# chenkovsky/aha

Hardware: AMD Instinct MI355X
Metric: input GB/s scanned + M-hits/s, 100k-pattern AC over 1 GiB UTF-8 corpus (higher is better)
Workload: dtype u8

## Files before the change

### aha_amd/csrc/scan_unit.hip

```cpp
#include <hip/hip_runtime.h>

#include "automaton.hpp"
#include "devcommon.hpp"
#include "image.hpp"
#include "unit.hpp"

namespace aha {

namespace {

constexpr int kUPiece = 16;
constexpr int kUWin = 3 * kUPiece;
constexpr int kURow = kUWin + 4;
constexpr int kUWave = 64 * kURow;

__device__ __forceinline__ uint4 load16(const uint8_t *text, int64_t g, int64_t N) {
  uint4 v = make_uint4(0, 0, 0, 0);
  if (g >= 0 && g + 16 <= N) {
    v = *reinterpret_cast<const uint4 *>(text + g);
  } else if (g >= 0 && g < N) {
    uint32_t w0 = 0, w1 = 0, w2 = 0, w3 = 0;
#pragma unroll 1
    for (int j = 0; j < 16 && g + j < N; j++) {
      const uint32_t b = (uint32_t)text[g + j] << ((j & 3) * 8);
      w0 |= (j >> 2) == 0 ? b : 0u;
      w1 |= (j >> 2) == 1 ? b : 0u;
      w2 |= (j >> 2) == 2 ? b : 0u;
      w3 |= (j >> 2) == 3 ? b : 0u;
    }
    v = make_uint4(w0, w1, w2, w3);
  }
  return v;
}

__device__ __forceinline__ uint64_t wballot(bool p) { return __builtin_amdgcn_ballot_w64(p); }
__device__ __forceinline__ bool wany(bool p) { return __builtin_amdgcn_ballot_w64(p) != 0ull; }
__device__ __forceinline__ bool wall(bool p) { return __builtin_amdgcn_ballot_w64(!p) == 0ull; }

__host__ __device__ inline size_t u_lds_rows(uint32_t n_syms) {
  return (size_t)(kUTabWords + ((n_syms + 3u) & ~3u)) * 4 + (size_t)(kV2Threads / 64) * kUWave + 16;
}
__host__ __device__ inline size_t u_lds(uint32_t n_syms) {
  return u_lds_rows(n_syms) + (size_t)(kV2Threads / 64) * 64 * 12;
}

template <bool CHARS, int BB, bool HB>
__global__ __launch_bounds__(kV2Threads) void ku_traverse(UnitDev U, V2Args M) {
  extern __shared__ __attribute__((aligned(16))) uint8_t smem[];
  if (M.cursor[1] >= 16ull) return;
  uint32_t *tabw = reinterpret_cast<uint32_t *>(smem);
  uint32_t *rlw = tabw + kUTabWords;
  const uint32_t n_root = (U.n_syms + 3u) & ~3u;
  for (uint32_t i = threadIdx.x; i < kUTabWords; i += kV2Threads) tabw[i] = U.tables[i];
  for (uint32_t i = threadIdx.x; i < n_root; i += kV2Threads) rlw[i] = i < U.n_syms ? U.root[i] : 0u;
  __syncthreads();
  const uint32_t *rl = rlw;
  const uint4 *t0a = reinterpret_cast<const uint4 *>(tabw + kUT0a);
  const uint2 *t0b = reinterpret_cast<const uint2 *>(tabw + kUT0b);
  const uint8_t *tabb = reinterpret_cast<const uint8_t *>(tabw);
  uint8_t *in_base = smem + (size_t)(kUTabWords + n_root) * 4;
  const int lane = threadIdx.x & 63, wave = threadIdx.x >> 6;
  uint8_t *inl = in_base + wave * kUWave + lane * kURow;
  const uint32_t *row = reinterpret_cast<const uint32_t *>(inl);
  typedef uint32_t v3u __attribute__((ext_vector_type(3)));
  const uint32_t wbo = (uint32_t)u_lds_rows(U.n_syms) + (uint32_t)wave * (64u * 12u);
  const uint2 *slots = U.slots;
  const int64_t N = (int64_t)M.n_bytes;
  const uint64_t D = M.n_docs;
  const int64_t S = (int64_t)M.S;
  const int rounds = (int)(M.S / kUPiece);
  const int warm = U.max_len > 1 ? (int)U.max_len - 1 : 0;
  const int R = (warm + kUPiece - 1) / kUPiece;

  const uint64_t n_tiles = (M.n_chunks + kV2Threads - 1) / kV2Threads;
  for (uint64_t tile = blockIdx.x; tile < n_tiles; tile += gridDim.x) {
    const uint64_t chunk = tile * kV2Threads + threadIdx.x;
    const uint32_t ev_stride = M.ev_stride;
    const bool live = chunk < M.n_chunks;
    const int64_t a = (int64_t)chunk * S;
    const int64_t e = live ? min(a + S, N) : a;
    uint64_t dn = 0;
    int64_t nb = INT64_MAX, doc_start = a, pos = e;
    uint32_t wfill = 0, wout = 0;
    const uint64_t wchunk0 = tile * kV2Threads + (uint64_t)wave * 64;
    uint32_t *wreg = M.evg + wchunk0 * M.ev_stride * 3;
    const uint32_t wcap = (uint32_t)min<uint64_t>(64, M.n_chunks > wchunk0 ? M.n_chunks - wchunk0 : 0) * M.ev_stride;
    uint32_t hits = 0;
    uint32_t lead_total = 0;
    uint32_t lc = 0, lc_exact = 0;
    uint32_t E = 0, seq = 0;
    uint32_t pc = 0;
    uint4 q1 = make_uint4(0, 0, 0, 0), q2 = q1, q3 = q1;
    uint32_t w[13] = {0, 0, 0, 0, 0, 0, 0, 0, 0, 0, 0, 0, 0};
    if (live) {
      dn = first_boundary(M.doc_off, D, (uint64_t)a);
      nb = (int64_t)M.doc_off[dn];
      pos = a;
      if (nb != a) {
        doc_start = (int64_t)M.doc_off[dn - 1];
        pos = a - min<int64_t>(a - doc_start, warm);
        if (CHARS) M.chunk_doc0[chunk] = (uint32_t)(dn - 1);
      } else if (CHARS) {
        M.chunk_doc0[chunk] = (uint32_t)dn;
      }
    }

    for (int r = -((R + 3) / 4) * 4 - 2; r <= rounds; r++) {
      const int64_t pb = a + (int64_t)r * kUPiece;
      const int64_t pl = pb + 2 * kUPiece;
      const int64_t pend = min(pb + kUWin, e);
      {
        uint4 v;
        if ((pl & 63) == 0) {
          v = load16(M.text, pl, N);
          q1 = load16(M.text, pl + 16, N);
          q2 = load16(M.text, pl + 32, N);
          q3 = load16(M.text, pl + 48, N);
        } else {
          v = q1;
          q1 = q2;
          q2 = q3;
        }
#pragma unroll
        for (int i = 0; i < 9; i++) w[i] = w[i + 4];
        w[9] = v.x;
        w[10] = v.y;
        w[11] = v.z;
        w[12] = v.w;
        uint32_t *dst = reinterpret_cast<uint32_t *>(inl);
#pragma unroll
        for (int i = 0; i < 13; i++) dst[i] = w[i];
      }
      const bool need = live && pos < pend;
      if (!wany(need)) continue;
      uint32_t rel = kURow, lim = 0;
      if (need) {
        rel = (uint32_t)(pos - pb + 4);
        lim = (uint32_t)(pend - pb + 4);
      }
      uint32_t nb_rel = (nb >= pb - 4 && nb <= pb + kUWin) ? (uint32_t)(nb - pb + 4) : ~0u;
      const uint32_t n_rel = (N - pb) <= (int64_t)kUWin ? (uint32_t)max<int64_t>(N - pb + 4, 0) : ~0u;
      const int32_t a_rel = (int32_t)max<int64_t>(a - pb + 4, -128);
      const int32_t e_rel = (int32_t)min<int64_t>(e - pb + 4, 128);
      int32_t docrel = (int32_t)(pb - 4 - doc_start);

      for (;;) {
        const bool bnd = rel < lim && rel == nb_rel;
        if (wany(bnd)) {
          if (bnd) {
            const int64_t here = pb - 4 + rel;
            do {
              M.doc_ev_rank[dn] = seq;
              M.doc_hit_rank[dn] = hits;
              if (CHARS) M.doc_lead_rank[dn] = lead_total;
              dn++;
              nb = dn <= D ? (int64_t)M.doc_off[dn] : INT64_MAX;
            } while (nb == here);
            asm volatile("" : "+v"(nb));
            nb_rel = (nb <= pb + kUWin) ? (uint32_t)(nb - pb + 4) : ~0u;
            E = 0;
            pc = 0;
            lc = 0;
            lc_exact = 1;
            doc_start = here;
            docrel = -(int32_t)rel;
          }
        }
        uint32_t lim2 = min(lim, nb_rel);
        const uint32_t dend = min(nb_rel, n_rel);
        auto decode = [&](uint32_t at, uint32_t &o_code, uint32_t &o_L, bool &o_later) {
          const uint32_t lo = row[at >> 2], hi = row[(at >> 2) + 1];
          const uint32_t w4 = __builtin_amdgcn_alignbyte(hi, lo, at & 3u);
          const uint32_t b0 = w4 & 0xFFu;
          const uint4 q0 = t0a[b0];
          const uint2 q1 = t0b[b0];
          const uint32_t s1 = *reinterpret_cast<const uint32_t *>(tabb + q0.x + ((w4 >> 6) & 0x3FCu));
          const uint32_t s2 = *reinterpret_cast<const uint32_t *>(tabb + q0.y + ((w4 >> 14) & 0x3FCu));
          const uint32_t sum = q0.z + s1 + s2;
          const uint32_t want = q1.y;
          const bool in_doc = at + want <= dend;
          o_later = in_doc & at + want > (uint32_t)kURow;
          const bool whole = in_doc & sum < kUPoison;
          const bool o_good = whole & (sum - q0.w) < q1.x;
          o_L = whole ? want : 1u;
          if (CHARS) o_L |= (b0 & 0xC0u) != 0x80u ? 0x100u : 0u;
          o_code = o_good ? sum - kUBias : 0u;
        };
        uint32_t code, L;
        {
          bool later;
          decode(min(rel, (uint32_t)kURow), code, L, later);
          lim2 = later ? min(lim2, rel) : lim2;
          lim = later ? min(lim, rel) : lim;
        }
        bool all_left = false;
        for (;;) {
          const bool act = rel < lim2;
          all_left = wall(rel >= (uint32_t)(4 + kUPiece) || rel >= lim);
          if (all_left || !wany(act)) break;
          auto trip = [&]() -> uint32_t {
            uint32_t evc = 0;
            const bool good = code != 0u;
            const uint32_t Bq = u_child(E, BB);
            const bool hdr = u_hdr_pending(E);
            const bool grp = Bq >= U.big_lo & code >= U.n_low & !hdr;
            uint32_t se = grp ? (code >> 5) + U.g0 : code;
            se = hdr ? 0u : se;
            const uint32_t fc = BB == 22 ? (code & 7u) : min(code & 7u, 6u);
            const bool probe = act & good & (((E | 0x20000000u) >> ((uint32_t)BB + fc)) & 1u) != 0u & Bq != 0u;
            unsigned long long enw = 0;
            uint32_t hdw = 0;
            {
              const uint2 *ap = slots + (probe ? (Bq ^ se) : 0u);
              asm volatile("global_load_dwordx2 %0, %1, off" : "=v"(enw) : "v"(ap) : "memory");
              if (HB) {
                const uint2 *hp = slots + ((act & u_nfr(E) & !u_f1(E)) ? Bq : 0u);
                asm volatile("global_load_dword %0, %1, off" : "=v"(hdw) : "v"(hp) : "memory");
              }
            }
            if (act) {
              uint32_t n_code, n_L;
              bool n_later;
              const uint32_t Lb = CHARS ? (L & 0xFFu) : L;
              decode(rel + Lb, n_code, n_L, n_later);
              const uint32_t rt = rl[code];
              const uint32_t rf = rl[pc];
              if (HB)
                asm volatile("s_waitcnt vmcnt(0)" : "+v"(enw), "+v"(hdw) : : "memory");
              else
                asm volatile("s_waitcnt vmcnt(0)" : "+v"(enw) : : "memory");
              const uint32_t enx = (uint32_t)enw, eny = (uint32_t)(enw >> 32);
              const bool symhit = probe & u_sym(eny) == se & !grp;
              const bool hit = symhit & !hdr;
              const bool redir = grp & probe & ((enx >> (code & 31u)) & 1u) != 0u;
              const uint32_t rE = (__builtin_popcount(enx & ~(~0u << (code & 31u))) + eny ^ code) | u_all_filter(BB);
              const bool viaroot = !symhit & !redir & (!u_nfr(E) | !good);
              const uint32_t ft = u_f1(E) ? (rf & 0x7FFFFFFFu) : (HB ? hdw : (Bq | u_all_filter(BB) | 0x20000000u));
              uint32_t missE = viaroot ? rt : ft;
              missE = redir ? rE : missE;
              E = symhit ? enx : missE;
              const bool consumed = hit | viaroot;
              const bool end = consumed & u_end(E);
              const uint32_t c4 = hit ? u_c4(eny) : 1u;
              pc = consumed ? code : pc;
              const uint32_t adv = consumed ? Lb : 0u;
              if (CHARS) {
                const uint32_t isl = (consumed & (int32_t)rel >= a_rel) ? (L >> 8) : 0u;
                lc += isl;
                lead_total += isl;
              }
              rel += adv;
              const bool park = consumed & n_later;
              lim2 = park ? rel : lim2;
              lim = park ? rel : lim;
              code = consumed ? n_code : code;
              L = consumed ? n_L : L;
              const int32_t last = (int32_t)rel - 1;
              evc = (end & last >= a_rel & last < e_rel) ? c4 : 0u;
            }
            return evc;
          };
          const uint32_t evc = trip();
          const uint64_t evm = wballot(evc != 0u);
          if (evm) {
            const bool ev = evc != 0u;
            const uint32_t my = wfill + __builtin_amdgcn_mbcnt_hi((uint32_t)(evm >> 32), __builtin_amdgcn_mbcnt_lo((uint32_t)evm, 0u));
            const uint32_t rx = u_rec_x(u_child(E, BB), (uint32_t)lane, evc, BB), rz = u_rec_z(hits, evc, BB);
            const uint32_t ry = CHARS ? ((lc << 1) | lc_exact) : (uint32_t)(docrel + (int32_t)rel);
            if (ev && my < 64u) {
              uint32_t *d = reinterpret_cast<uint32_t *>(smem + (wbo + __umul24(my, 12u)));
              d[0] = rx;
              d[1] = ry;
              d[2] = rz;
            }
            const uint32_t kp = __popcll(evm);
            if (wfill + kp >= 64u) {
              const uint32_t *q = reinterpret_cast<const uint32_t *>(smem + (wbo + __umul24((uint32_t)lane, 12u)));
              const v3u r = {q[0], q[1], q[2]};
#ifndef AHA_KU_LAB_NOFLUSH
              if (wout + 64u <= wcap) *reinterpret_cast<v3u *>(wreg + (size_t)(wout + lane) * 3) = r;
#else
              if (wout + 64u == 0xFFFFFFF0u) *reinterpret_cast<v3u *>(wreg + (size_t)(wout + lane) * 3) = r;
#endif
              wout += 64u;
              if (ev && my >= 64u) {
                uint32_t *d = reinterpret_cast<uint32_t *>(smem + (wbo + __umul24(my - 64u, 12u)));
                d[0] = rx;
                d[1] = ry;
                d[2] = rz;
              }
            }
            wfill = (wfill + kp) & 63u;
            seq += ev ? 1u : 0u;
            hits += evc;
          }
        }
        if (all_left || !wany(rel < lim)) break;
      }
      if (need) pos = pb - 4 + rel;
    }
    {
      const uint32_t *q = reinterpret_cast<const uint32_t *>(smem + (wbo + __umul24((uint32_t)lane, 12u)));
      const v3u r = {q[0], q[1], q[2]};
      if ((uint32_t)lane < wfill && wout + (uint32_t)lane < wcap) *reinterpret_cast<v3u *>(wreg + (size_t)(wout + lane) * 3) = r;
    }
    if (live) {
      M.ev_cnt[chunk] = seq;
      if (seq > ev_stride) M.cursor[1] = 2ull;
      if (CHARS) M.lead_cnt[chunk] = lead_total;
      M.chunk_hits[chunk] = hits;
      if (e == N) {
        while (dn <= D) {
          M.doc_ev_rank[dn] = seq;
          M.doc_hit_rank[dn] = hits;
          if (CHARS) M.doc_lead_rank[dn] = lead_total;
          dn++;
        }
      }
    }
  }
}

constexpr int kRgThreads = 256, kRgPer = 4, kRgBlock = kRgThreads * kRgPer, kRgSubs = kRgBlock / 64;
__global__ __launch_bounds__(kRgThreads) void ku_regroup(DevAut A, V2Args M) {
  __shared__ uint2 s_sorted[kRgBlock];
  __shared__ uint8_t s_lane[kRgBlock];
  __shared__ uint32_t s_cnt[kRgSubs][64], s_part[kRgThreads / 64][64];
  __shared__ uint32_t s_start[64], s_tot[64], s_run[64], s_hits[64];
  if (M.cursor[1]) return;
  const int lane = threadIdx.x & 63, wv = threadIdx.x >> 6;
  const uint64_t n_groups = (M.n_chunks + 63) / 64;
  const uint32_t stride = M.ev_stride;
  const uint32_t bb = M.unit_bb, bmask = (1u << bb) - 1u;
  for (uint64_t g = blockIdx.x; g < n_groups; g += gridDim.x) {
    __syncthreads();
    if (wv == 0) {
      s_run[lane] = 0;
      s_hits[lane] = 0;
    }
    const uint64_t c = g * 64 + lane;
    uint32_t total = c < M.n_chunks ? min(M.ev_cnt[c], stride) : 0u;
#pragma unroll
    for (int d = 32; d >= 1; d >>= 1) total += __shfl_xor(total, d, 64);
    const uint32_t *src = M.evg + g * 64 * stride * 3;
    uint2 *dst = M.evd + g * 64 * stride;
    uint2 nxt[kRgPer];
    uint32_t xn[kRgPer];
#pragma unroll
    for (int q = 0; q < kRgPer; q++) {
      const uint32_t i = q * kRgThreads + threadIdx.x;
      nxt[q] = i < total ? make_uint2(src[(size_t)i * 3], src[(size_t)i * 3 + 1]) : make_uint2(0, 0);
    }
#pragma unroll
    for (int q = 0; q < kRgPer; q++) xn[q] = (uint32_t)(q * kRgThreads) + threadIdx.x < total ? A.end_info[nxt[q].x & bmask] : 0u;
    for (uint32_t i0 = 0; i0 < total; i0 += kRgBlock) {
      uint2 rec[kRgPer];
      uint32_t x[kRgPer], rank[kRgPer], l[kRgPer];
      bool live[kRgPer];
#pragma unroll
      for (int q = 0; q < kRgPer; q++) {
        const uint32_t i = i0 + q * kRgThreads + threadIdx.x;
        live[q] = i < total;
        rec[q] = nxt[q];
        x[q] = xn[q];
        nxt[q] = i + kRgBlock < total ? make_uint2(src[(size_t)(i + kRgBlock) * 3], src[(size_t)(i + kRgBlock) * 3 + 1])
                                      : make_uint2(0, 0);
      }
#pragma unroll
      for (int q = 0; q < kRgPer; q++) {
        l[q] = (rec[q].x >> bb) & 63u;
        uint64_t same = __ballot(live[q]), mine = same;
#pragma unroll
        for (int b = 0; b < 6; b++) {
          const uint64_t bal = __ballot(live[q] & ((l[q] >> b) & 1u) != 0u);
          same &= ((l[q] >> b) & 1u) ? bal : ~bal;
          mine &= ((lane >> b) & 1) ? bal : ~bal;
        }
        rank[q] = __popcll(same & ((1ull << lane) - 1ull));
        s_cnt[q * (kRgThreads / 64) + wv][lane] = __popcll(mine);
      }
      __syncthreads();
      {
        uint32_t acc = 0;
#pragma unroll
        for (int r = 0; r < kRgSubs / (kRgThreads / 64); r++) {
          const uint32_t v = s_cnt[wv * (kRgSubs / (kRgThreads / 64)) + r][lane];
          s_cnt[wv * (kRgSubs / (kRgThreads / 64)) + r][lane] = acc;
          acc += v;
        }
        s_part[wv][lane] = acc;
      }
      __syncthreads();
      if (wv == 0) {
        uint32_t acc = 0;
#pragma unroll
        for (int w2 = 0; w2 < kRgThreads / 64; w2++) {
          const uint32_t v = s_part[w2][lane];
          s_part[w2][lane] = acc;
          acc += v;
        }
        s_tot[lane] = acc;
        s_start[lane] = wave_incl_scan(acc) - acc;
      }
      __syncthreads();
#pragma unroll
      for (int q = 0; q < kRgPer; q++) {
        if (live[q]) {
          const uint32_t sb = q * (kRgThreads / 64) + wv;
          const uint32_t p = s_start[l[q]] + s_part[sb / (kRgSubs / (kRgThreads / 64))][l[q]] + s_cnt[sb][l[q]] + rank[q];
          uint32_t cnt = x[q] >> 24;
          if (cnt == 255u) cnt = A.key_cnt[A.chain ? A.chain[x[q] & 0xFFFFFFu].y : (x[q] & 0xFFFFFFu)];
          s_sorted[p] = make_uint2(x[q], rec[q].y);
          s_lane[p] = (uint8_t)l[q];
          if (cnt) atomicAdd(&s_hits[l[q]], cnt);
        }
      }
      __syncthreads();
#pragma unroll
      for (int q = 0; q < kRgPer; q++)
        xn[q] = i0 + kRgBlock + (uint32_t)(q * kRgThreads) + threadIdx.x < total ? A.end_info[nxt[q].x & bmask] : 0u;
#pragma unroll
      for (int q = 0; q < kRgPer; q++) asm volatile("" : "+v"(xn[q]));
      const uint32_t nb = min(total - i0, (uint32_t)kRgBlock);
#pragma unroll
      for (int q = 0; q < kRgPer; q++) {
        const uint32_t p = q * kRgThreads + threadIdx.x;
        if (p < nb) {
          const uint32_t lp = s_lane[p];
          const uint32_t at = s_run[lp] + (p - s_start[lp]);
          if (at < stride) dst[(uint64_t)lp * stride + at] = s_sorted[p];
        }
      }
      __syncthreads();
      if (wv == 0) s_run[lane] += s_tot[lane];
    }
    __syncthreads();
    if (wv == 0 && c < M.n_chunks) M.chunk_hits[c] = s_hits[lane];
  }
}

constexpr int kXgThreads = 1024, kXgPer = 1, kXgBlock = kXgThreads * kXgPer, kXgStage = 1536;
constexpr int kXgCacheBits = 11;
template <bool CHARS>
__global__ __launch_bounds__(kXgThreads) void ku_expand_groups(const uint2 *uend, DevAut A, V2Args M) {
  __shared__ uint32_t s_hs[kXgStage], s_he[kXgStage], s_hk[kXgStage];
  __shared__ uint8_t s_hl[kXgStage];
  __shared__ uint32_t s_tot[2][64], s_start[64], s_run[64], s_all;
  __shared__ uint64_t s_base[64];
  __shared__ uint32_t s_adj[64];
  __shared__ unsigned long long s_cache[1 << kXgCacheBits];
  if (M.cursor[1]) return;
  const int lane = threadIdx.x & 63, wv = threadIdx.x >> 6;
  const uint64_t n_groups = (M.n_chunks + 63) / 64;
  const uint32_t stride = M.ev_stride;
  const uint32_t bb = M.unit_bb, bmask = (1u << bb) - 1u;
  for (uint32_t i = threadIdx.x; i < (1u << kXgCacheBits); i += kXgThreads) s_cache[i] = 0ull;
  for (uint64_t g = blockIdx.x; g < n_groups; g += gridDim.x) {
    __syncthreads();
    const uint64_t c = g * 64 + lane;
    if (wv == 0) {
      if (CHARS && c < M.n_chunks) s_adj[lane] = M.lead_cnt[c];
      s_base[lane] = c < M.n_chunks ? M.hit_base[c] : 0ull;
      s_run[lane] = 0;
      s_tot[0][lane] = 0;
    }
    uint32_t total = c < M.n_chunks ? min(M.ev_cnt[c], stride) : 0u;
#pragma unroll
    for (int d = 32; d >= 1; d >>= 1) total += __shfl_xor(total, d, 64);
    const uint32_t *src = M.evg + g * 64 * stride * 3;
    typedef uint32_t v3u __attribute__((ext_vector_type(3)));
    v3u nxt[kXgPer];
#pragma unroll
    for (int q = 0; q < kXgPer; q++) {
      const uint32_t i = q * kXgThreads + threadIdx.x;
      nxt[q] = i < total ? __builtin_nontemporal_load(reinterpret_cast<const v3u *>(src + (size_t)i * 3)) : v3u{0, 0, 0};
    }
    __syncthreads();
    uint32_t par = 0;
    for (uint32_t i0 = 0; i0 < total; i0 += kXgBlock, par ^= 1u) {
      v3u rec[kXgPer];
      uint2 ue[kXgPer];
      bool live[kXgPer], keep[kXgPer];
      uint32_t cs[kXgPer];
#pragma unroll
      for (int q = 0; q < kXgPer; q++) {
        const uint32_t i = i0 + q * kXgThreads + threadIdx.x;
        live[q] = i < total;
        rec[q] = nxt[q];
        nxt[q] = i + kXgBlock < total ? __builtin_nontemporal_load(reinterpret_cast<const v3u *>(src + (size_t)(i + kXgBlock) * 3)) : v3u{0, 0, 0};
        const uint32_t b = rec[q].x & bmask, n = u_rec_n(rec[q].x, rec[q].z, bb);
        cs[q] = (b * 0x9E3779B1u) >> (32 - kXgCacheBits);
        const unsigned long long ce = s_cache[cs[q]];
        const bool cached = live[q] & n == 1u & (uint32_t)ce == b + 1u;
        ue[q] = make_uint2((uint32_t)(ce >> 32), 0u);
        if (live[q] && !cached) ue[q] = uend[b];
        keep[q] = live[q] & !cached & n == 1u;
        if (live[q]) atomicAdd(&s_tot[par][(rec[q].x >> bb) & 63u], n);
      }
      __syncthreads();
      if (wv == 0) {
        const uint32_t t = s_tot[par][lane];
        const uint32_t incl = wave_incl_scan(t);
        s_start[lane] = incl - t;
        if (lane == 63) s_all = incl;
        s_tot[par ^ 1u][lane] = 0;
      }
      __syncthreads();
      const uint32_t T = s_all;
#pragma unroll
      for (int q = 0; q < kXgPer; q++)
        if (keep[q] && (ue[q].y >> 24) == 0u)
          atomicExch(&s_cache[cs[q]], (unsigned long long)ue[q].x << 32 | ((rec[q].x & bmask) + 1u));
      for (uint32_t w0 = 0; w0 < T; w0 += kXgStage) {
#pragma unroll
        for (int q = 0; q < kXgPer; q++) {
          if (live[q]) {
            const uint32_t l = (rec[q].x >> bb) & 63u, n = u_rec_n(rec[q].x, rec[q].z, bb);
            const uint32_t pos = s_start[l] + (u_rec_before(rec[q].z) - s_run[l]);
            const uint32_t end = CHARS ? (rec[q].y >> 1) + ((rec[q].y & 1u) ? 0u : s_adj[l]) : rec[q].y, co = ue[q].y & 0xFFFFFFu;
            uint32_t len = (ue[q].x >> 24) | (ue[q].y >> 24) << 8, key = ue[q].x & 0xFFFFFFu;
            for (uint32_t k = 0;;) {
              const uint32_t j = pos + k - w0;
              if (j < (uint32_t)kXgStage) {
                s_hs[j] = end - len;
                s_he[j] = end;
                s_hk[j] = key;
                s_hl[j] = (uint8_t)l;
              }
              if (++k >= n) break;
              const uint2 ce = (CHARS ? A.chain_chars : A.chain)[co + k];
              len = ce.x;
              key = ce.y;
            }
          }
        }
        __syncthreads();
        const uint32_t nh = min(T - w0, (uint32_t)kXgStage);
        for (uint32_t j = threadIdx.x; j < nh; j += kXgThreads) {
          const uint32_t l = s_hl[j];
          const uint64_t idx = s_base[l] + s_run[l] + (w0 + j - s_start[l]);
          if (idx < M.cap) {
            aha_hit hit;
            hit.start = (int32_t)s_hs[j];
            hit.end = (int32_t)s_he[j];
            hit.value = (int32_t)s_hk[j];
            M.out[idx] = hit;
          }
        }
        __syncthreads();
      }
      if (wv == 0) s_run[lane] += s_tot[par][lane];
    }
  }
}

__global__ __launch_bounds__(256) void ku_chunk_adj(V2Args M) {
  if (M.cursor[1]) return;
  const uint64_t c = (uint64_t)blockIdx.x * 256 + threadIdx.x;
  if (c >= M.n_chunks) return;
  const uint32_t d0 = M.chunk_doc0[c];
  const uint64_t dchunk = M.doc_off[d0] / M.S;
  M.lead_cnt[c] = (uint32_t)(M.lead_base[c] - (M.lead_base[dchunk] + M.doc_lead_rank[d0]));
}

__global__ __launch_bounds__(256) void ku_doc_offsets(V2Args M) {
  if (M.publish && blockIdx.x == 0 && threadIdx.x < 5) M.publish[threadIdx.x] = M.cursor[threadIdx.x];
  if (M.clear_next && blockIdx.x == 0 && threadIdx.x < 16) M.clear_next[threadIdx.x] = 0ull;
  if (M.cursor[1] || !M.doc_hit_off) return;
  const uint64_t d = (uint64_t)blockIdx.x * 256 + threadIdx.x;
  if (d > M.n_docs) return;
  const uint64_t q = M.doc_off[d];
  M.doc_hit_off[d] = q < M.n_bytes ? M.hit_base[q / M.S] + M.doc_hit_rank[d] : M.totals[0];
}

}

size_t unit_lds_bytes(uint32_t n_syms) { return u_lds(n_syms); }

int unit_prepare(uint32_t n_syms) {
  const int lds = (int)unit_lds_bytes(n_syms);
  int e = 0;
#define AHA_PREP_KU(C, B, H) \
  if (!e) e = (int)hipFuncSetAttribute((const void *)ku_traverse<C, B, H>, hipFuncAttributeMaxDynamicSharedMemorySize, lds);
  AHA_PREP_KU(false, 22, false) AHA_PREP_KU(true, 22, false) AHA_PREP_KU(false, 23, false) AHA_PREP_KU(true, 23, false)
  AHA_PREP_KU(false, 22, true) AHA_PREP_KU(true, 22, true) AHA_PREP_KU(false, 23, true) AHA_PREP_KU(true, 23, true)
#undef AHA_PREP_KU
  return e;
}

void unit_launch_traverse(const UnitDev &U, const V2Args &M, uint32_t grid, void *stream) {
  const size_t lds = unit_lds_bytes(U.n_syms);
#define AHA_LAUNCH_KU(C, B, H) hipLaunchKernelGGL((ku_traverse<C, B, H>), dim3(grid), dim3(kV2Threads), lds, (hipStream_t)stream, U, M)
#define AHA_LAUNCH_KU2(C, B) \
  do {                       \
    if (U.hdr_beside)        \
      AHA_LAUNCH_KU(C, B, true);  \
    else                     \
      AHA_LAUNCH_KU(C, B, false); \
  } while (0)
  if (U.base_bits == 23) {
    if (M.chars) AHA_LAUNCH_KU2(true, 23); else AHA_LAUNCH_KU2(false, 23);
  } else {
    if (M.chars) AHA_LAUNCH_KU2(true, 22); else AHA_LAUNCH_KU2(false, 22);
  }
#undef AHA_LAUNCH_KU2
#undef AHA_LAUNCH_KU
}

void unit_launch_doc_offsets(const V2Args &M, void *stream) {
  if (M.doc_hit_off)
    hipLaunchKernelGGL(ku_doc_offsets, dim3((uint32_t)((M.n_docs + 1 + 255) / 256)), dim3(256), 0, (hipStream_t)stream, M);
}

void unit_launch_regroup(const DevAut &A, const V2Args &M, void *stream) {
  const uint64_t n_groups = (M.n_chunks + 63) / 64;
  hipLaunchKernelGGL(ku_regroup, dim3((uint32_t)std::min<uint64_t>(n_groups, 1u << 16)), dim3(kRgThreads), 0,
                     (hipStream_t)stream, A, M);
}

void unit_launch_expand(const uint2 *uend, const DevAut &A, const V2Args &M, uint32_t workgroups, void *stream) {
  const uint64_t n_groups = (M.n_chunks + 63) / 64;
  const dim3 grid((uint32_t)std::max<uint64_t>(1, std::min<uint64_t>(n_groups, workgroups)));
  if (M.chars) {
    hipLaunchKernelGGL(ku_chunk_adj, dim3((uint32_t)((M.n_chunks + 255) / 256)), dim3(256), 0, (hipStream_t)stream, M);
    hipLaunchKernelGGL(ku_expand_groups<true>, grid, dim3(kXgThreads), 0, (hipStream_t)stream, uend, A, M);
  } else {
    hipLaunchKernelGGL(ku_expand_groups<false>, grid, dim3(kXgThreads), 0, (hipStream_t)stream, uend, A, M);
  }
  if (M.doc_hit_off)
    hipLaunchKernelGGL(ku_doc_offsets, dim3((uint32_t)((M.n_docs + 1 + 255) / 256)), dim3(256), 0, (hipStream_t)stream, M);
}

}
```

Before: 440.1.

## Rebase scan loop to 32-bit chunk-relative offsets and carry decode state across rounds

Replaces per-round 64-bit position arithmetic with 32-bit offsets relative to the chunk start, wave-uniform base addresses and a carried rel counter. Adds a fast path doing unchecked 64-byte vector loads when the whole wave is inside the buffer. Skips re-decoding the current symbol at round entry when it is still valid from the previous round. This cuts scalar/VALU integer overhead in the hot loop, but the warm-up start round changes and the stale-decode carry adds correctness risk at boundaries.

```diff
diff --git a/aha_amd/csrc/scan_unit.hip b/aha_amd/csrc/scan_unit.hip
--- a/aha_amd/csrc/scan_unit.hip
+++ b/aha_amd/csrc/scan_unit.hip
@@ -13,16 +13,17 @@
 constexpr int kUWin = 3 * kUPiece;
 constexpr int kURow = kUWin + 4;
 constexpr int kUWave = 64 * kURow;
-
-__device__ __forceinline__ uint4 load16(const uint8_t *text, int64_t g, int64_t N) {
+constexpr int32_t kUFar = 1 << 30;
+
+__device__ __forceinline__ uint4 load16(const uint8_t *p, int32_t front, int32_t left) {
   uint4 v = make_uint4(0, 0, 0, 0);
-  if (g >= 0 && g + 16 <= N) {
-    v = *reinterpret_cast<const uint4 *>(text + g);
-  } else if (g >= 0 && g < N) {
+  if (front >= 0 && left >= 16) {
+    v = *reinterpret_cast<const uint4 *>(p);
+  } else if (front >= 0 && left > 0) {
     uint32_t w0 = 0, w1 = 0, w2 = 0, w3 = 0;
 #pragma unroll 1
-    for (int j = 0; j < 16 && g + j < N; j++) {
-      const uint32_t b = (uint32_t)text[g + j] << ((j & 3) * 8);
+    for (int j = 0; j < left; j++) {
+      const uint32_t b = (uint32_t)p[j] << ((j & 3) * 8);
       w0 |= (j >> 2) == 0 ? b : 0u;
       w1 |= (j >> 2) == 1 ? b : 0u;
       w2 |= (j >> 2) == 2 ? b : 0u;
@@ -59,7 +60,7 @@
   const uint2 *t0b = reinterpret_cast<const uint2 *>(tabw + kUT0b);
   const uint8_t *tabb = reinterpret_cast<const uint8_t *>(tabw);
   uint8_t *in_base = smem + (size_t)(kUTabWords + n_root) * 4;
-  const int lane = threadIdx.x & 63, wave = threadIdx.x >> 6;
+  const int lane = threadIdx.x & 63, wave = __builtin_amdgcn_readfirstlane((int)(threadIdx.x >> 6));
   uint8_t *inl = in_base + wave * kUWave + lane * kURow;
   const uint32_t *row = reinterpret_cast<const uint32_t *>(inl);
   typedef uint32_t v3u __attribute__((ext_vector_type(3)));
@@ -71,18 +72,21 @@
   const int rounds = (int)(M.S / kUPiece);
   const int warm = U.max_len > 1 ? (int)U.max_len - 1 : 0;
   const int R = (warm + kUPiece - 1) / kUPiece;
+  const int r0 = -R - 2;
+  const uint32_t la = (uint32_t)lane * (uint32_t)M.S;
 
   const uint64_t n_tiles = (M.n_chunks + kV2Threads - 1) / kV2Threads;
   for (uint64_t tile = blockIdx.x; tile < n_tiles; tile += gridDim.x) {
     const uint64_t chunk = tile * kV2Threads + threadIdx.x;
     const uint32_t ev_stride = M.ev_stride;
     const bool live = chunk < M.n_chunks;
-    const int64_t a = (int64_t)chunk * S;
+    const uint64_t wchunk0 = tile * kV2Threads + (uint64_t)wave * 64;
+    const int64_t wa = (int64_t)wchunk0 * S;
+    const int64_t a = wa + (int64_t)la;
     const int64_t e = live ? min(a + S, N) : a;
     uint64_t dn = 0;
     int64_t nb = INT64_MAX, doc_start = a, pos = e;
     uint32_t wfill = 0, wout = 0;
-    const uint64_t wchunk0 = tile * kV2Threads + (uint64_t)wave * 64;
     uint32_t *wreg = M.evg + wchunk0 * M.ev_stride * 3;
     const uint32_t wcap = (uint32_t)min<uint64_t>(64, M.n_chunks > wchunk0 ? M.n_chunks - wchunk0 : 0) * M.ev_stride;
     uint32_t hits = 0;
@@ -104,18 +108,50 @@
         M.chunk_doc0[chunk] = (uint32_t)dn;
       }
     }
-
-    for (int r = -((R + 3) / 4) * 4 - 2; r <= rounds; r++) {
-      const int64_t pb = a + (int64_t)r * kUPiece;
-      const int64_t pl = pb + 2 * kUPiece;
-      const int64_t pend = min(pb + kUWin, e);
+    const int32_t e_off = (int32_t)(e - a);
+    const int32_t n_off = N - a < (int64_t)kUFar ? (int32_t)(N - a) : kUFar;
+    int32_t nb_off = nb - a <= S + kUWin ? (int32_t)(nb - a) : kUFar;
+    int32_t docbase = (int32_t)(a - doc_start);
+    uint32_t rel = live ? (uint32_t)((int32_t)(pos - a) - (16 * r0 - 4) + 16) : (uint32_t)kUFar;
+    uint32_t code = 0, L = 1;
+    bool stale = true;
+    const int32_t wa_s = wa < (int64_t)kUFar ? (int32_t)wa : kUFar;
+    const int64_t hi = N - 64 - 63 * S - wa;
+    const int32_t po_lo = -wa_s, po_hi = hi < (int64_t)kUFar ? (hi > -(int64_t)kUFar ? (int32_t)hi : -kUFar) : kUFar;
+    const int32_t front = wa_s + (int32_t)la;
+    if (((r0 + 2) & 3) != 0) {
+      const int j = (r0 + 2) & 3;
+      const int32_t po = 16 * (r0 + 2 - j);
+      const uint8_t *p = M.text + (wa + po) + la;
+      q1 = load16(p + 16, front + po + 16, n_off - po - 16);
+      q2 = load16(p + 32, front + po + 32, n_off - po - 32);
+      q3 = load16(p + 48, front + po + 48, n_off - po - 48);
+      if (j >= 2) {
+        q1 = q2;
+        q2 = q3;
+      }
+      if (j == 3) q1 = q2;
+    }
+
+    for (int r = r0; r <= rounds; r++) {
+      const int32_t c = 16 * r - 4;
+      const int32_t po = 16 * r + 32;
       {
         uint4 v;
-        if ((pl & 63) == 0) {
-          v = load16(M.text, pl, N);
-          q1 = load16(M.text, pl + 16, N);
-          q2 = load16(M.text, pl + 32, N);
-          q3 = load16(M.text, pl + 48, N);
+        if ((po & 63) == 0) {
+          if (po >= po_lo && po <= po_hi) {
+            const uint4 *p = reinterpret_cast<const uint4 *>(M.text + (wa + po) + la);
+            v = p[0];
+            q1 = p[1];
+            q2 = p[2];
+            q3 = p[3];
+          } else {
+            const uint8_t *p = M.text + (wa + po) + la;
+            v = load16(p, front + po, n_off - po);
+            q1 = load16(p + 16, front + po + 16, n_off - po - 16);
+            q2 = load16(p + 32, front + po + 32, n_off - po - 32);
+            q3 = load16(p + 48, front + po + 48, n_off - po - 48);
+          }
         } else {
           v = q1;
           q1 = q2;
@@ -131,24 +167,25 @@
 #pragma unroll
         for (int i = 0; i < 13; i++) dst[i] = w[i];
       }
-      const bool need = live && pos < pend;
+      rel -= (uint32_t)kUPiece;
+      const int32_t e_row = e_off - c;
+      const int32_t lim_r = min(e_row, (int32_t)kURow);
+      const bool need = (int32_t)rel < lim_r;
       if (!wany(need)) continue;
-      uint32_t rel = kURow, lim = 0;
-      if (need) {
-        rel = (uint32_t)(pos - pb + 4);
-        lim = (uint32_t)(pend - pb + 4);
-      }
-      uint32_t nb_rel = (nb >= pb - 4 && nb <= pb + kUWin) ? (uint32_t)(nb - pb + 4) : ~0u;
-      const uint32_t n_rel = (N - pb) <= (int64_t)kUWin ? (uint32_t)max<int64_t>(N - pb + 4, 0) : ~0u;
-      const int32_t a_rel = (int32_t)max<int64_t>(a - pb + 4, -128);
-      const int32_t e_rel = (int32_t)min<int64_t>(e - pb + 4, 128);
-      int32_t docrel = (int32_t)(pb - 4 - doc_start);
+      uint32_t lim = need ? (uint32_t)lim_r : 0u;
+      uint32_t nb_rel = (uint32_t)(nb_off - c);
+      nb_rel = nb_rel <= (uint32_t)kURow ? nb_rel : ~0u;
+      const int32_t n_row = n_off - c;
+      const uint32_t n_rel = n_row <= (int32_t)kURow ? (uint32_t)max(n_row, 0) : ~0u;
+      const int32_t a_rel = max(-c, -128);
+      const int32_t e_rel = min(e_row, 128);
+      int32_t docrel = docbase + c;
 
       for (;;) {
         const bool bnd = rel < lim && rel == nb_rel;
         if (wany(bnd)) {
           if (bnd) {
-            const int64_t here = pb - 4 + rel;
+            const int64_t here = a + (int64_t)(c + (int32_t)rel);
             do {
               M.doc_ev_rank[dn] = seq;
               M.doc_hit_rank[dn] = hits;
@@ -157,13 +194,16 @@
               nb = dn <= D ? (int64_t)M.doc_off[dn] : INT64_MAX;
             } while (nb == here);
             asm volatile("" : "+v"(nb));
-            nb_rel = (nb <= pb + kUWin) ? (uint32_t)(nb - pb + 4) : ~0u;
+            nb_off = nb - a <= S + kUWin ? (int32_t)(nb - a) : kUFar;
+            nb_rel = (uint32_t)(nb_off - c);
+            nb_rel = nb_rel <= (uint32_t)kURow ? nb_rel : ~0u;
+            stale = true;
             E = 0;
             pc = 0;
             lc = 0;
             lc_exact = 1;
-            doc_start = here;
             docrel = -(int32_t)rel;
+            docbase = docrel - c;
           }
         }
         uint32_t lim2 = min(lim, nb_rel);
@@ -186,8 +226,7 @@
           if (CHARS) o_L |= (b0 & 0xC0u) != 0x80u ? 0x100u : 0u;
           o_code = o_good ? sum - kUBias : 0u;
         };
-        uint32_t code, L;
-        {
+        if (wany(stale & rel < lim)) {
           bool later;
           decode(min(rel, (uint32_t)kURow), code, L, later);
           lim2 = later ? min(lim2, rel) : lim2;
@@ -297,7 +336,7 @@
         }
         if (all_left || !wany(rel < lim)) break;
       }
-      if (need) pos = pb - 4 + rel;
+      stale = rel >= lim;
     }
     {
       const uint32_t *q = reinterpret_cast<const uint32_t *>(smem + (wbo + __umul24((uint32_t)lane, 12u)));
@@ -309,7 +348,7 @@
       if (seq > ev_stride) M.cursor[1] = 2ull;
       if (CHARS) M.lead_cnt[chunk] = lead_total;
       M.chunk_hits[chunk] = hits;
-      if (e == N) {
+      if (e_off == n_off) {
         while (dn <= D) {
           M.doc_ev_rank[dn] = seq;
           M.doc_hit_rank[dn] = hits;
```

New measurement: 443.2 (median of 3 runs). No clear change (+0.7%).
